# visinf/da-sac

Measured on AMD Instinct MI355X. Metric: train images/sec (769x769, 19-cls, RN101 DeepLabv2, K=3), higher is better.
Workload: dtype f32

## Files before the change

da-sac_amd/csrc/winograd.hip:

```cpp
#include "conv_common.hpp"
#include "winograd_index.hpp"

namespace dasac {
namespace wino {

constexpr int kBlock = 256;

__device__ __forceinline__ float ld(__amdgpu_buffer_rsrc_t r, unsigned voff) {
  return __uint_as_float(__builtin_amdgcn_raw_buffer_load_b32(r, voff, 0, 0));
}
__device__ __forceinline__ void st(__amdgpu_buffer_rsrc_t r, unsigned voff, float v) {
  __builtin_amdgcn_raw_buffer_store_b32(__float_as_uint(v), r, voff, 0, 0);
}

__global__ __launch_bounds__(kBlock) void filter_transform(const float* __restrict__ Wt, const float* __restrict__ scale,
                                                            float* __restrict__ U, int Cout, int Cin, int Mpad, int Kpad, int mode,
                                                            unsigned w_bytes, unsigned u_bytes) {
  const int idx = blockIdx.x * kBlock + threadIdx.x;
  const int per_point = Kpad * Mpad;
  if (idx >= per_point) return;
  const __amdgpu_buffer_rsrc_t rw = make_rsrc(Wt, w_bytes), ru = make_rsrc(U, u_bytes);
  const int row4 = Mpad * 4;
  const int kq = idx / row4, rem = idx - kq * row4;
  const int m = rem >> 2, k = kq * 4 + (rem & 3);
// ... 303 lines not shown
    float r[3][6];
#pragma unroll
    for (int b = 0; b < 6; ++b) {
      float p[6], o[3];
#pragma unroll
      for (int a = 0; a < 6; ++a) p[a] = (red[0][a * 6 + b][c] + red[1][a * 6 + b][c]) + (red[2][a * 6 + b][c] + red[3][a * 6 + b][c]);
      gt3(p[0], p[1], p[2], p[3], p[4], p[5], o);
#pragma unroll
      for (int a = 0; a < 3; ++a) r[a][b] = o[a];
    }
#pragma unroll
    for (int a = 0; a < 3; ++a) {
      float o[3];
      gt3(r[a][0], r[a][1], r[a][2], r[a][3], r[a][4], r[a][5], o);
#pragma unroll
      for (int b = 0; b < 3; ++b) grad[c * 9 + a * 3 + b] = o[b];
    }
  }
  __syncthreads();
  const float sc = scale ? ld(make_rsrc(scale, (unsigned)M * 4u), (unsigned)co * 4u) : 1.f;
  float part = 0.f;
  for (int e = tx; e < 64 * 9; e += kBlock) {
    const unsigned off = ((unsigned)(co * C + ci0) * 9u + (unsigned)e) * 4u;
    if (dot) part += grad[e] * ld(rw, off);
    st(rd, off, grad[e] * sc);
  }
  if (dot) {
    __shared__ float redd[4];
    part = wave_sum(part);
    if (c == 0) redd[q] = part;
    __syncthreads();
    if (tx == 0) st(make_rsrc(dot, (unsigned)((C / 64) * M) * 4u), (unsigned)(blockIdx.x * M + co) * 4u, (redd[0] + redd[1]) + (redd[2] + redd[3]));
  }
}

}
}

using namespace dasac;
using dasac::wino::Geom;

static int wino_geom(Geom& g, const char* who, int Nb, int C, int M, int H, int W, int dilation) {
  DASAC_REQUIRE(Nb > 0 && C > 0 && M > 0 && H > 0 && W > 0 && dilation > 0, "%s: bad geometry", who);
  DASAC_REQUIRE((int64_t)Nb * H * W < (1ll << 30), "%s: more than 2^30 pixels", who);
  g = wino::make_geom(Nb, H, W, dilation);
  const int64_t cmax = C > M ? C : M;
  DASAC_REQUIRE(16 * cmax * (int64_t)g.T * 4 <= wino::kMaxBytes && cmax * (int64_t)Nb * H * W * 4 <= wino::kMaxBytes,
                "%s: a tensor exceeds the 4 GiB buffer-descriptor window", who);
  return DASAC_OK;
}

extern "C" int dasac_winograd_tiles(int Nb, int H, int W, int dilation) {
  if (Nb <= 0 || H <= 0 || W <= 0 || dilation <= 0) return 0;
  const int64_t t = (int64_t)Nb * wino::make_axis(H, dilation).tiles * wino::make_axis(W, dilation).tiles;
  return t < (1ll << 30) ? (int)t : 0;
}

extern "C" int dasac_winograd_filter(const float* w, const float* scale, int Cout, int Cin, int transposed, float* u,
                                     dasac_stream_t stream) {
  DASAC_REQUIRE(w && u, "winograd_filter: null pointer");
  DASAC_REQUIRE(Cout > 0 && Cin > 0, "winograd_filter: bad channel counts");
  const int M = transposed ? Cin : Cout, K = transposed ? Cout : Cin;
  const int Mpad = dasac_conv_mpad(M), Kpad = dasac_conv_kpad(K);
  const int64_t per_point = (int64_t)Kpad * Mpad;
  DASAC_REQUIRE(16 * per_point * 4 <= wino::kMaxBytes && (int64_t)Cout * Cin * 9 * 4 <= wino::kMaxBytes,
                "winograd_filter: operand exceeds the 4 GiB buffer-descriptor window");
// ... 112 lines not shown
}

extern "C" int dasac_winograd4_grad_input(const float* dz, int Nb, int M, int H, int W, int dilation, float* dm, size_t dm_bytes,
                                          dasac_stream_t stream) {
  DASAC_REQUIRE(dz && dm, "winograd4_grad_input: null pointer");
  Geom g;
  const int rc = wino_geom4(g, "winograd4_grad_input", Nb, M, H, W, dilation);
  if (rc) return rc;
  const size_t need = (size_t)36 * M * g.T * 4;
  if (dm_bytes < need) return fail(DASAC_EWORKSPACE, "winograd4_grad_input: workspace too small (%zu < %zu)", dm_bytes, need);
  hipLaunchKernelGGL(wino::grad_transform4, dim3((g.T + wino::kBlock - 1) / wino::kBlock, M), dim3(wino::kBlock), 0, as_stream(stream), dz,
                     dm, g, M, (unsigned)((int64_t)Nb * M * H * W * 4), (unsigned)need);
  DASAC_CHECK_LAUNCH("winograd grad_transform4");
  return DASAC_OK;
}

extern "C" int dasac_winograd4_wgrad_finish(const void* workspace, size_t ws_bytes, int M, int C, int T, const float* w,
                                            const float* scale, float* dw, float* dot, float* sum_dz, dasac_stream_t stream) {
  DASAC_REQUIRE(workspace && w && dw, "winograd4_wgrad_finish: null pointer");
  DASAC_REQUIRE(M > 0 && M <= 65535 && C > 0 && C % 64 == 0, "winograd4_wgrad_finish: needs 1..65535 output channels and a multiple of 64 input channels");
  const int splits = dasac_conv_wgrad_batched_splits(36, M, C, T);
  DASAC_REQUIRE(splits > 0, "winograd4_wgrad_finish: the batched weight-gradient launch does not take this shape");
  const size_t need = dasac_conv_wgrad_batched_workspace(36, M, C, T);
  if (ws_bytes < need) return fail(DASAC_EWORKSPACE, "winograd4_wgrad_finish: workspace too small (%zu < %zu)", ws_bytes, need);
  const int64_t p_elems = (int64_t)splits * 36 * M * C;
  DASAC_REQUIRE(p_elems * 4 <= wino::kMaxBytes && (int64_t)M * C * 9 * 4 <= wino::kMaxBytes,
                "winograd4_wgrad_finish: a tensor exceeds the 4 GiB buffer-descriptor window");
  const float* P = reinterpret_cast<const float*>(workspace);
  hipLaunchKernelGGL(wino::wgrad_finish4, dim3(C / 64, M), dim3(wino::kBlock), 0, as_stream(stream), P, P + p_elems, splits, M, C, w, scale,
                     dw, dot, sum_dz, (unsigned)(p_elems * 4), (unsigned)((int64_t)M * C * 9 * 4));
  DASAC_CHECK_LAUNCH("winograd wgrad_finish4");
  return DASAC_OK;
}
```

da-sac_amd/csrc/winograd_index.hpp:

```cpp
#pragma once
#include <stdint.h>

#if defined(__HIPCC__)
#define DASAC_HD __host__ __device__ __forceinline__
#else
#define DASAC_HD inline
#endif

namespace dasac {
namespace wino {

struct Div {
  unsigned mul, shift;
  int d;
};
DASAC_HD Div make_div(int d) {
  Div f{0u, 0u, d < 1 ? 1 : d};
  if (d <= 1) return f;
  int l = 1;
  while ((1ll << l) < d) ++l;
  const unsigned long long p = 1ull << (31 + l);
  f.mul = (unsigned)((p + (unsigned)d - 1) / (unsigned)d);
  f.shift = (unsigned)(l - 1);
  return f;
// ... 70 lines not shown
}
template <int TM = 2>
DASAC_HD void tile_origin(const Geom& g, int tile, int& n, int& y0, int& x0) {
  n = div(tile, g.by_tiles_img);
  const int rem = tile - n * g.tiles_img;
  const int gy = div(rem, g.by_tx), gx = rem - gy * g.ax.tiles;
  int p, t;
  tile_decode(g.ay, gy, p, t);
  y0 = first_out<TM>(g.ay, p, t);
  tile_decode(g.ax, gx, p, t);
  x0 = first_out<TM>(g.ax, p, t);
}
DASAC_HD bool real_tile(const Geom& g, int tile) { return tile < g.N * g.tiles_img; }
template <int TM = 2>
DASAC_HD void pixel_tile(const Geom& g, int pix, int& n, int& rem, int& tile, int& ey, int& ex) {
  n = div(pix, g.by_hw);
  rem = pix - n * g.HW;
  const int y = div(rem, g.by_w), x = rem - y * g.W;
  int gy, gx;
  coord_to_tile<TM>(g.ay, y, gy, ey);
  coord_to_tile<TM>(g.ax, x, gx, ex);
  tile = (n * g.ay.tiles + gy) * g.ax.tiles + gx;
}

constexpr unsigned kOutside = 0xFFFFFFFFu;

DASAC_HD unsigned patch_offset(const Geom& g, int C, int n, int c, int y0, int x0, int ky, int kx) {
  const int y = y0 + (ky - 1) * g.ay.d, x = x0 + (kx - 1) * g.ax.d;
  if ((unsigned)y >= (unsigned)g.H || (unsigned)x >= (unsigned)g.W) return kOutside;
  return (unsigned)((n * C + c) * g.HW + y * g.W + x) * 4u;
}
DASAC_HD unsigned point_offset(const Geom& g, int C, int pt, int c, int tile) { return (unsigned)((pt * C + c) * g.T + tile) * 4u; }
DASAC_HD unsigned out_offset(const Geom& g, int M, int n, int m, int rem) { return (unsigned)((n * M + m) * g.HW + rem) * 4u; }
constexpr int64_t kMaxBytes = (1ll << 32) - 4096;

}
}
```

da-sac_amd/dasac_hip/engine.py:

```python
import torch

from . import ops
from . import lib as L


class ConvOp:
    kind = "conv"

    def __init__(self, src, dst, convs, bn, relu, res):
        c0 = convs[0]
        self.src, self.dst, self.res, self.relu = src, dst, res, bool(relu)
        self.convs, self.bn = list(convs), bn
        assert all(c.stride == c0.stride and c.in_channels == c0.in_channels and c.out_channels == c0.out_channels
                   and c.groups == 1 for c in convs)
        assert c0.stride[0] == c0.stride[1]
        branches = []
        for c in convs:
            assert c.dilation[0] == c.dilation[1] and c.padding[0] == c.padding[1]
            branches.append((c.kernel_size[0], c.kernel_size[1], c.dilation[0], c.padding[0]))
        self.spec = ops.ConvSpec(c0.in_channels, c0.out_channels, branches, c0.stride[0])
        self.has_bias = c0.bias is not None
        assert bn is None or len(convs) == 1
        self.expanded = ops.ExpandedConv(self.spec) if (len(convs) > 1 and c0.out_channels <= 32 and c0.stride[0] == 1) else None

# ... 25 lines not shown
        return self.expanded is None and len(self.convs) == 1

    def inputs(self):
        return [self.src] + ([self.res] if self.res is not None else [])

    def tensors(self, c, h, w):
        oh, ow = self.spec.out_hw(h, w)
        return ([(self.expanded.E, oh, ow)] if self.expanded is not None else []) + [(self.spec.cout, oh, ow)]

    def forward(self, eng, i, saved, keep):
        acts, spec = saved["acts"], self.spec
        xin = acts[self.src]
        Nb, _, H, W = xin.shape
        if self.expanded is not None:
            _, bias_sum, _ = eng.fold(self)
            return self.expanded.forward(xin, eng.packed(self, False), eng.table(self, H, W, False, xin.device), bias_sum)
        OH, OW = spec.out_hw(H, W)
        out = torch.empty((Nb, spec.cout, OH, OW), dtype=torch.float32, device=xin.device)
        res = None if self.res is None else acts[self.res]
        if self.bn is not None and self.bn.training:
            cb = self.convs[0].bias.detach() if self.has_bias else None
            ts = ops.tile_stats_buffer(Nb, spec.cout, OH, OW, xin.device) if ops.stats_ok(spec.cout, spec.cin) else None
            z = ops.conv_gemm(xin, eng.packed(self, False, None), eng.table(self, H, W, False, xin.device), out, (OH, OW),
                              spec.stride, spec.cout, spec.K, 1, cb, None, None, False, stats=ts)
            out, stats = ops.bn_train_forward(z, self.bn, res, self.relu, tile_stats=ts)
            if keep:
                saved["aux"][i] = (z, stats)
            return out
        scale, shift, _ = eng.fold(self)
        bits = None
        if keep and self.relu and eng._bits_wanted[self.dst] and ops.bits_ok(spec.cout, spec.cin):
            bits = ops.ReluBits(Nb, spec.cout, OH, OW, xin.device)
            saved["bits"][self.dst] = bits
        if res is None and ops.winograd_routed(spec, False, Nb, H, W):
            return ops.winograd_conv(xin, eng.winograd_filter(self, False, scale), out, spec.branches[0][2], shift, self.relu,
                                     bits_out=bits)
        return ops.conv_gemm(xin, eng.packed(self, False, scale), eng.table(self, H, W, False, xin.device), out, (OH, OW),
                             spec.stride, spec.cout, spec.K, 1, shift, res, None, self.relu, bits_out=bits)

    def backward(self, eng, bp, i, dz):
        spec, ex = self.spec, self.expanded
        xin = bp.acts[self.src]
        H, W = xin.shape[2:]
        dy_out = dz
        if ex is not None:
            d = ex.scatter(dz)
            self._param_grads_expanded(eng, bp, d, dz, xin)
        else:
            dz, scale = self._param_grads(eng, bp, i, dz, xin)
        if self.src != 0:
            relu = bp.arrive(self.src)
            if ex is not None:
                mask = bp.relu_pattern(self.src, spec.cin, ex.E) if relu else None
                bp.g[self.src] = ex.dgrad(d, eng.packed(self, True), eng.table(self, H, W, True, dz.device), (H, W),
                                          res=bp.g.get(self.src), mask=mask)
            else:
                mask = (bp.relu_pattern(self.src, spec.cin, spec.cout) if spec.stride == 1 else bp.acts[self.src]) if relu else None
                OH, OW = dz.shape[2:]
                if bp.g.get(self.src) is None and (mask is None or isinstance(mask, ops.ReluBits)) \
                        and ops.winograd_routed(spec, True, dz.shape[0], OH, OW):
                    dx = torch.empty((dz.shape[0], spec.cin, H, W), dtype=torch.float32, device=dz.device)
                    bp.g[self.src] = ops.winograd_conv(dz, eng.winograd_filter(self, True, scale), dx, spec.branches[0][2],
                                                       mask_bits=mask)
                else:
                    bp.g[self.src] = ops.conv_dgrad(spec, dz, None, (H, W), scale=scale, res=bp.g.get(self.src), mask=mask,
                                                    table=eng.table(self, OH, OW, True, dz.device),
                                                    packed=eng.packed(self, True, scale))
        if self.res is not None:
            bp.join(self.res, dy_out)
        if bp.sink is not None:
            bp.sink.done([j for j in self.pidx if bp.need[j]])

    def _param_grads_expanded(self, eng, bp, d, dz, xin):
        need = bp.need
        if any(need[j] for j in self.w_idx):
            bp.store(self.w_idx, self.expanded.wgrad(d, xin, [c.weight.detach() for c in self.convs],
                                                     eng.table(self, xin.shape[2], xin.shape[3], False, xin.device),
                                                     outs=[bp.dest(j) for j in self.w_idx]))
        if any(need[j] for j in self.b_idx):
            bp.fan_out(self.b_idx, ops.channel_sums(dz, out=bp.sums_dest(self.b_idx, True, self.spec.cout, dz.device)))

    def _param_grads(self, eng, bp, i, dz, xin):
        spec, need, grads = self.spec, bp.need, bp.grads
        w_idx, b_idx, bn_idx = self.w_idx, self.b_idx, self.bn_idx
        train_bn = i in bp.aux
        want_bias = any(need[j] for j in b_idx)
        want_bn = any(need[j] for j in bn_idx)
        if train_bn:
            z, stats = bp.aux.pop(i)
            dz, dg, db = ops.bn_train_backward(dz, z, stats, self.bn.weight.detach(), want_params=want_bn,
                                               outs=(bp.dest(bn_idx[0]), bp.dest(bn_idx[1])) if want_bn else (None, None))
            del z
            if want_bn:
# ... 343 lines not shown
    @staticmethod
    def _cached(store, slot, key, build, *args):
        ent = store.get(slot)
        if ent is None or ent[0] != key:
            ent = store[slot] = (key, build(None if ent is None else ent[1], *args), args)
        return ent[1]

    def fold(self, op):
        if op.bn is None and (not op.has_bias or len(op.convs) == 1):
            return None, (op.convs[0].bias.detach() if op.has_bias else None), None
        return self._cached(self._folds, id(op), _fold_key(op), self._build_fold, op)

    @staticmethod
    def _build_fold(old, op):
        if op.bn is None:
            acc = op.convs[0].bias.detach()
            for c in op.convs[1:]:
                acc = ops.add(acc, c.bias.detach())
            return None, acc, None
        bn = op.bn
        return ops.bn_fold(bn.weight.detach(), bn.bias.detach(), bn.running_mean, bn.running_var, bn.eps,
                           op.convs[0].bias.detach() if op.has_bias else None)

    def packed(self, op, transposed, scale=None):
        return self._cached(self._packs, (id(op), transposed), _pack_key(op, scale), self._build_pack, op, transposed, scale)

    @staticmethod
    def _build_pack(old, op, transposed, scale):
        weights = [c.weight.detach() for c in op.convs]
        if op.expanded is not None:
            return op.expanded.pack(weights, transposed, out=old)
        return ops.conv_pack(op.spec, weights, transposed, scale, out=old, order=ops.gemm_order(op.spec, transposed))

    def winograd_filter(self, op, transposed, scale=None):
        return self._cached(self._packs, (id(op), transposed, "winograd"), _pack_key(op, scale), self._build_winograd_filter,
                            op, transposed, scale)

    @staticmethod
    def _build_winograd_filter(old, op, transposed, scale):
        return ops.winograd_filter(op.spec, op.convs[0].weight.detach(), transposed, scale, out=old)

    def largest_tensor_bytes(self, Nb, H, W):
        shapes = {0: (None, H, W)}
        biggest = 0
        for op in self.plan.ops:
            made = op.tensors(*shapes[op.src])
            shapes[op.dst] = made[-1]
            biggest = max([biggest] + [Nb * (c or 1) * h * w * 4 for c, h, w in made])
        return biggest

    def _refresh_plan(self, device, transposed):
        bn_mode = tuple(bool(op.bn is not None and op.bn.training) for op in self._convs)
        key = (device.index, bool(transposed), bn_mode)
        plan = self._refresh.get(key)
        if plan is not None and plan["ptrs"] == self._refresh_ptrs():
            return plan
        lib = L.load()
        fold_jobs, pack_jobs, fold_ops, pack_slots = [], [], [], []
        for op in self._convs:
            if not op.refreshable:
                continue
            scale = None
            if op.frozen_bn:
                ent = self._fold_bufs.get(id(op))
                if ent is None:
                    C = op.spec.cout
                    ent = tuple(torch.empty(C, dtype=torch.float32, device=device) for _ in range(3))
                    self._fold_bufs[id(op)] = ent
                scale = ent[0]
                cb = op.convs[0].bias if op.has_bias else None
                fold_jobs.append((op.bn.weight, op.bn.bias, op.bn.running_mean, op.bn.running_var, cb, ent, op.bn.eps, op.spec.cout))
                fold_ops.append(op)
            for tr in ((False, True) if transposed else (False,)):
# ... 257 lines not shown
```

da-sac_amd/dasac_hip/lib.py:

```python
import ctypes as C
import os

import torch

LIB_PATH = os.environ.get("DASAC_LIB") or os.path.join(os.path.dirname(os.path.abspath(__file__)), "libdasac_hip.so")

_p, _i, _l, _f, _sz = C.c_void_p, C.c_int, C.c_int64, C.c_float, C.c_size_t

PROTOTYPES = {
    "dasac_version": (_i, []),
    "dasac_last_error": (C.c_char_p, []),
    "dasac_device_info": (_i, [C.POINTER(_i), C.POINTER(_i), C.c_char_p, _sz]),
    "dasac_reserved_cus": (_i, []),
    "dasac_set_reserved_cus": (_i, [_i]),
    "dasac_pseudo_labels_workspace": (_sz, [_i, _i, _l]),
    "dasac_pseudo_labels": (_i, [_p, _p, _p, _f, _f, _i, _i, _l, _p, _p, _p, _p, _sz, _p]),
    "dasac_conv_mpad": (_i, [_i]),
    "dasac_conv_kpad": (_i, [_i]),
    "dasac_conv_table": (_i, [_p, _p, _p, _p, _i, _i, _i, _i, _i, _i, _p, _p]),
    "dasac_conv_pack": (_i, [_p, _p, _i, _i, _i, _i, _i, _i, _i, _p, _p]),
    "dasac_relu_bits_words": (_sz, [_i, _l]),
    "dasac_conv_gemm_bits_ok": (_i, [_i, _i]),
    "dasac_conv_gemm": (_i, [_p, _p, _p, _p] + [_i] * 12 + [_p, _p, _p, _p, _p, _i, _i, _i, _i, _p, _sz, _p]),
    "dasac_conv_gemm_batched": (_i, [_p, _p, _p, _p] + [_i] * 12 + [_i, _l, _l, _l, _p]),
# ... 40 lines not shown
    "dasac_activation_stats": (_i, [_p, _i, _i, _i, _p, _i, _p, _sz, _p, _p]),
    "dasac_label_nodes": (_i, [_p, _i, _i, _i, _i, _i, _i, _i, _i, _p, _p]),
    "dasac_class_feature_stats_workspace": (_sz, [_i, _i, _i]),
    "dasac_class_feature_stats": (_i, [_p, _p, _i, _i, _i, _i, _p, _p, _p, _sz, _p]),
    "dasac_scale_planes": (_i, [_p, _p, _l, _l, _p, _p]),
    "dasac_add": (_i, [_p, _p, _p, _l, _p]),
    "dasac_relu_mask": (_i, [_p, _p, _p, _l, _p]),
    "dasac_bn_stats_workspace": (_sz, [_i, _i, _l]),
    "dasac_bn_stats": (_i, [_p, _i, _i, _l, _p, _p, _sz, _p]),
    "dasac_bn_train_finalize": (_i, [_p, C.c_double, _p, _p, _p, _p, _p, _p, _f, _f, _i, _p, _p, _p, _p, _p]),
    "dasac_bn_apply": (_i, [_p, _p, _p, _p, _i, _i, _i, _l, _p, _p]),
    "dasac_bn_bwd_reduce": (_i, [_p, _p, _p, _p, _i, _i, _l, _p, _p, _p, _p, _sz, _p]),
    "dasac_bn_train_finalize_tiles": (_i, [_p, _i, _i, C.c_double, _p, _p, _p, _p, _p, _f, _f, _i, _p, _p, _p, _p, _p]),
    "dasac_bn_tile_stats_reduce": (_i, [_p, _i, _i, _i, _p, _p]),
    "dasac_bn_train_apply_tiles": (_i, [_p, _p, _i, _i, C.c_double, _p, _p, _p, _p, _p, _f, _f, _p, _i, _i, _i, _l, _p, _p, _p, _p]),
    "dasac_bn_bwd_fused": (_i, [_p, _p, _p, _p, _p, C.c_double, _i, _i, _l, _p, _p, _p, _p, _sz, _p]),
    "dasac_conv_gemm_stats_ok": (_i, [_i, _i]),
    "dasac_conv_gemm_stats_tiles": (_i, [_i, _i, _i]),
    "dasac_conv_gemm_stats": (_i, [_p, _p, _p, _p] + [_i] * 12 + [_p, _p, _i, _i, _i, _i, _p, _sz, _p, _p]),
    "dasac_bn_bwd_apply": (_i, [_p, _p, _p, _p, _p, _p, C.c_double, _p, _i, _i, _l, _p, _p, _p, _p]),
    "dasac_winograd_tiles": (_i, [_i, _i, _i, _i]),
    "dasac_winograd_filter": (_i, [_p, _p, _i, _i, _i, _p, _p]),
    "dasac_winograd_input": (_i, [_p, _i, _i, _i, _i, _i, _p, _sz, _p]),
    "dasac_winograd_output": (_i, [_p, _sz, _i, _i, _i, _i, _i, _p, _i, _p, _p, _p, _p]),
    "dasac_winograd_grad_input": (_i, [_p, _i, _i, _i, _i, _i, _p, _sz, _p]),
    "dasac_conv_wgrad_batched_splits": (_i, [_i, _i, _i, _i]),
    "dasac_conv_wgrad_batched_workspace": (_sz, [_i, _i, _i, _i]),
    "dasac_conv_wgrad_batched": (_i, [_p, _p, _i, _i, _i, _i, _l, _l, _i, _p, _sz, _p]),
    "dasac_winograd_wgrad_finish": (_i, [_p, _sz, _i, _i, _i, _p, _p, _p, _p, _p, _p]),
    "dasac_winograd4_tiles": (_i, [_i, _i, _i, _i]),
    "dasac_winograd4_input": (_i, [_p, _i, _i, _i, _i, _i, _p, _sz, _p]),
    "dasac_winograd4_grad_input": (_i, [_p, _i, _i, _i, _i, _i, _p, _sz, _p]),
    "dasac_winograd4_wgrad_finish": (_i, [_p, _sz, _i, _i, _i, _p, _p, _p, _p, _p, _p]),
    "dasac_conv_pack_expanded":(_i, [_p, _i, _i, _i, _i, _i, _i, _i, _p, _p]),
    "dasac_tap_gather": (_i, [_p, _p, _p, _p, _p, _i, _i, _i, _p, _i, _i, _i, _p, _p]),
    "dasac_tap_scatter": (_i, [_p, _p, _p, _p, _p, _i, _i, _i, _i, _i, _i, _p, _p]),
    "dasac_conv_wgrad_finish_expanded": (_i, [_p, _i, _i, _i, _i, _i, _p, _i, _i, _i, _i, _p]),
    "dasac_pack_chunk_elems": (_i, []),
    "dasac_bn_fold_multi": (_i, [_p, _p, _i, _p]),
    "dasac_conv_pack_multi": (_i, [_p, _p, _i, _p]),
    "dasac_label_pad_mask": (_i, [_p, _p, _l, _i, _i, _p]),
    "dasac_dropout_planes": (_i, [C.c_uint64, C.c_uint64, _f, _l, _p, _p]),
    "dasac_iou_counts": (_i, [_p, _p, _i, _i, _l, _i, _p, _p]),
    "dasac_mask_counts": (_i, [_p, _p, _p, _p, _p, _p, _p, _i, _i, _l, _i, _p, _p]),
    "dasac_confusion_counts": (_i, [_p, _p, _p, _p, _p, _p, _i, _p, _i, _i, _l, _i, _p, _p, _i, _i, _p]),
    "dasac_view_consistency": (_i, [_p, _i, _i, _i, _l, _f, _p, _p, _p, _p]),
    "dasac_boundary_counts_workspace": (_sz, [_i, _i, _i, _i]),
    "dasac_boundary_counts": (_i, [_p, _p, _p, _p, _p, _p, _i, _p, _i, _i, _i, _i, _i, _i, _p, _p, _sz, _p]),
    "dasac_crf_meanfield_workspace": (_sz, [_i, _i, _i, _i, _i]),
    "dasac_crf_meanfield": (_i, [_p, _p, _i, _i, _i, _i, _i, _i, _i, _f, _f, _f, _f, _f, _f, _i, _p, _p, _p, _p, _p, _sz, _p]),
    "dasac_label_hist": (_i, [_p, _i, _l, _p, _p]),
    "dasac_make_views_table_ints": (_i, [_i, _i]),
    "dasac_make_views": (_i, [_p, _p, _p, _i, _i, _i, _p, _p, _p, _i, _p, _p, _p, _p]),
    "dasac_view_photometric_workspace": (_sz, [_i, _i, _i]),
    "dasac_view_photometric": (_i, [_p, _p, _i, _i, _i, _p, _p, _p, _i, _p, _p, _p, _sz, _p]),
    "dasac_conv_wgrad_dot_rows": (_i, [_i, _i]),
    "dasac_conv_wgrad_finish": (_i, [_p, _i, _i, _i, _i, _i, _p, _p, _p, _p, _p, _i, _i, _i, _p]),
    "dasac_crop_table_ints": (_i, [_i, _i]),
    "dasac_resize_u8": (_i, [_p, _l, _p, _l, _i, _p, _p, _l, _i, _p, _l, _p, _l, _p]),
    "dasac_make_crops": (_i, [_p, _l, _p, _l, _i, _p, _p, _l, _i, _i, _p, _p, _i, _p, _p, _p, _p, _p, _p]),
    "dasac_vis_panels": (_i, [_p, _p, _i, _i, _i, _i, _i, _p, _p, _p, _p, _p, _p, _p]),
    "dasac_vis_grid": (_i, [_p, _i, _i, _i, _i, _f, _p, _p]),
}


class VisJob(C.Structure):
# ... 106 lines not shown
```

da-sac_amd/dasac_hip/ops.py:

```python
import os

import torch

from . import lib as L


def _c(t):
    return t if t.is_contiguous() else t.contiguous()


class _Profile:

    def __init__(self):
        self.on, self.records = False, []

    def start(self):
        self.on, self.records = True, []

    def stop(self, by_shape=False):
        self.on = False
        torch.cuda.synchronize()
        out = {}
        for name, flops, a, b, tag, nbytes in self.records:
            d = out.setdefault((name, tag) if by_shape else name, {"flops": 0.0, "bytes": 0.0, "seconds": 0.0, "launches": 0})
# ... 307 lines not shown
    with PROFILE.span("winograd_output", 0.0, None, 4.0 * (y.numel() + out.numel())):
        L.check(lib.dasac_winograd_output(y.data_ptr(), y.numel() * 4, Nb, M, H, W, int(dilation), L.ptr(shift), int(relu),
                                          0 if mask_bits is None else mask_bits.words.data_ptr(),
                                          0 if bits_out is None else bits_out.words.data_ptr(), out.data_ptr(), L.stream_ptr()),
                "dasac_winograd_output")
    return out


def winograd_conv(x, u, out, dilation, shift=None, relu=False, mask_bits=None, bits_out=None, gemm_schedule="auto"):
    lib = L.load()
    L.require_gpu(x, u, out)
    Nb, C, H, W = x.shape
    M = out.shape[1]
    assert x.is_contiguous() and out.is_contiguous() and tuple(out.shape) == (Nb, M, H, W)
    assert tuple(u.shape) == (16, lib.dasac_conv_kpad(C), lib.dasac_conv_mpad(M)) and u.is_contiguous()
    T = lib.dasac_winograd_tiles(Nb, H, W, int(dilation))
    if T <= 0 or 64 * max(C, M) * T > _MAX_TENSOR_BYTES:
        raise L.DasacError("winograd_conv: [16, {}, tiles] exceeds the 4 GiB buffer-descriptor window".format(max(C, M)))
    v_elems, y_elems = 16 * C * T, 16 * M * T
    ws = L.workspace(4 * (v_elems + y_elems), x.device)[:4 * (v_elems + y_elems)].view(torch.float32)
    v, y = ws[:v_elems].view(16, C, T), ws[v_elems:v_elems + y_elems].view(16, M, T)
    with PROFILE.span("winograd_input", 0.0, None, 4.0 * (x.numel() + v_elems)):
        L.check(lib.dasac_winograd_input(x.data_ptr(), Nb, C, H, W, int(dilation), v.data_ptr(), v_elems * 4, L.stream_ptr()),
                "dasac_winograd_input")
    table = _winograd_table(C, T, x.device)
    if gemm_schedule == "auto" and lib.dasac_conv_mpad(M) % 128 != 0:
        gemm_schedule = None
    if gemm_schedule == "auto":
        conv_gemm_batched(v.view(16, 1, C, 1, T), u, table, y.view(16, 1, M, 1, T), (1, T), 1, M, C)
    else:
        for pt in range(16):
            conv_gemm(v[pt].view(1, C, 1, T), u[pt], table, y[pt].view(1, M, 1, T), (1, T), 1, M, C, schedule=gemm_schedule)
    return winograd_output(y, out, dilation, shift, relu, mask_bits, bits_out)


WINOGRAD_WGRAD_MIN_CHANNEL_PRODUCT = 256 * 256


def winograd_wgrad_routed(spec, Nb, H, W):
    if ALGORITHM != "auto" or not winograd_ok(spec) or spec.cin * spec.cout < WINOGRAD_WGRAD_MIN_CHANNEL_PRODUCT:
        return False
    lib = L.load()
    T = lib.dasac_winograd_tiles(Nb, H, W, spec.branches[0][2])
    return T > 0 and 64 * max(spec.cin, spec.cout) * T <= _MAX_TENSOR_BYTES \
        and lib.dasac_conv_wgrad_batched_splits(16, spec.cout, spec.cin, T) > 0


def winograd_wgrad(spec, dz, x, weight, scale=None, dot=None, sum_dz=None, out=None):
    lib = L.load()
    L.require_gpu(dz, x, weight, scale, dot, sum_dz)
    Nb, C, H, W = x.shape
    M, d = dz.shape[1], int(spec.branches[0][2])
    assert winograd_ok(spec) and (C, M) == (spec.cin, spec.cout) and tuple(dz.shape) == (Nb, M, H, W) and x.is_contiguous()
    assert dot is None or (tuple(dot.shape) == (dot_rows(spec), M) and dot.is_contiguous())
    T = lib.dasac_winograd_tiles(Nb, H, W, d)
    slab_bytes = lib.dasac_conv_wgrad_batched_workspace(16, M, C, T) if T > 0 else 0
    if slab_bytes == 0 or 64 * max(C, M) * T > _MAX_TENSOR_BYTES:
        raise L.DasacError("winograd_wgrad: {} x {} channels over {} tiles has no batched point contraction".format(M, C, T))
    v_elems, m_elems = 16 * C * T, 16 * M * T
    ws = L.workspace(4 * (v_elems + m_elems) + slab_bytes, x.device)
    v, dm, slabs = ws[:4 * v_elems], ws[4 * v_elems:4 * (v_elems + m_elems)], ws[4 * (v_elems + m_elems):]
    dz = _c(dz)
    with PROFILE.span("winograd_wgrad_input", 0.0, None, 4.0 * (x.numel() + v_elems)):
        L.check(lib.dasac_winograd_input(x.data_ptr(), Nb, C, H, W, d, v.data_ptr(), v.numel(), L.stream_ptr()), "dasac_winograd_input")
    with PROFILE.span("winograd_wgrad_grad", 0.0, None, 4.0 * (dz.numel() + m_elems)):
        L.check(lib.dasac_winograd_grad_input(dz.data_ptr(), Nb, M, H, W, d, dm.data_ptr(), dm.numel(), L.stream_ptr()),
# ... 1126 lines not shown
```

include/dasac_hip.h:

```cpp
#ifndef DASAC_HIP_H
#define DASAC_HIP_H

#include <stddef.h>
#include <stdint.h>

#ifdef __cplusplus
extern "C" {
#endif

#define DASAC_OK 0
#define DASAC_EINVAL (-1)
#define DASAC_EWORKSPACE (-2)
#define DASAC_ELAUNCH (-3)

typedef void* dasac_stream_t;

int dasac_version(void);
const char* dasac_last_error(void);
int dasac_device_info(int* cu_count, int* wave_size, char* arch, size_t arch_len);
int dasac_reserved_cus(void);
int dasac_set_reserved_cus(int n);

size_t dasac_pseudo_labels_workspace(int B, int C, int64_t HW);
int dasac_pseudo_labels(const float* probs, const uint8_t* ignore, const float* disc,
// ... 44 lines not shown
int dasac_conv_wgrad(const float* dz, const float* x, const int32_t* table,
                     int Nb, int Cx, int H, int W, int OH, int OW, int stride, int M, int K,
                     void* workspace, size_t ws_bytes, dasac_stream_t stream);
int dasac_conv_wgrad_x3(const float* dz, const float* x, const int32_t* table,
                        int Nb, int Cx, int H, int W, int OH, int OW, int stride, int M, int K,
                        void* workspace, size_t ws_bytes, dasac_stream_t stream);
int dasac_conv_wgrad_dot_rows(int Cin, int taps);
int dasac_conv_wgrad_finish(const void* workspace, int Nb, int OH, int OW, int M, int K,
                            const float* w, const float* scale, float* dw, float* dot,
                            float* sum_dz, int Cin, int taps, int tap0, dasac_stream_t stream);

int dasac_winograd_tiles(int Nb, int H, int W, int dilation);
int dasac_winograd_filter(const float* w, const float* scale, int Cout, int Cin, int transposed, float* u,
                          dasac_stream_t stream);
int dasac_winograd_input(const float* x, int Nb, int C, int H, int W, int dilation, float* v, size_t v_bytes,
                         dasac_stream_t stream);
int dasac_winograd_output(const float* y, size_t y_bytes, int Nb, int M, int H, int W, int dilation, const float* shift,
                          int relu, const uint32_t* mask_bits, uint32_t* relu_bits_out, float* out, dasac_stream_t stream);
int dasac_winograd_grad_input(const float* dz, int Nb, int M, int H, int W, int dilation, float* dm, size_t dm_bytes,
                              dasac_stream_t stream);
int dasac_conv_wgrad_batched_splits(int batch, int M, int C, int T);
size_t dasac_conv_wgrad_batched_workspace(int batch, int M, int C, int T);
int dasac_conv_wgrad_batched(const float* a, const float* b, int batch, int M, int C, int T, int64_t a_stride, int64_t b_stride,
                             int sum_entry, void* workspace, size_t ws_bytes, dasac_stream_t stream);
int dasac_winograd_wgrad_finish(const void* workspace, size_t ws_bytes, int M, int C, int T, const float* w, const float* scale,
                                float* dw, float* dot, float* sum_dz, dasac_stream_t stream);
int dasac_winograd4_tiles(int Nb, int H, int W, int dilation);
int dasac_winograd4_input(const float* x, int Nb, int C, int H, int W, int dilation, float* v, size_t v_bytes,
                          dasac_stream_t stream);
int dasac_winograd4_grad_input(const float* dz, int Nb, int M, int H, int W, int dilation, float* dm, size_t dm_bytes,
                               dasac_stream_t stream);
int dasac_winograd4_wgrad_finish(const void* workspace, size_t ws_bytes, int M, int C, int T, const float* w, const float* scale,
                                 float* dw, float* dot, float* sum_dz, dasac_stream_t stream);

int dasac_conv_pack_expanded(const float* w, int Cout, int Cin, int taps, int tap0, int total_taps,
                             int Cp, int transposed, float* packed, dasac_stream_t stream);
int dasac_tap_gather(const float* y, const int32_t* kh, const int32_t* kw, const int32_t* dil,
                     const int32_t* pad, int n_branches, int Cp, int Cout, const float* bias, int B,
                     int H, int W, float* out, dasac_stream_t stream);
int dasac_tap_scatter(const float* dout, const int32_t* kh, const int32_t* kw, const int32_t* dil,
                      const int32_t* pad, int n_branches, int Cp, int Cout, int B, int H, int W,
                      float* d, dasac_stream_t stream);
int dasac_conv_wgrad_finish_expanded(const void* workspace, int Nb, int OH, int OW, int E, int Cin,
                                     float* dw, int Cout, int taps, int tap0, int Cp,
                                     dasac_stream_t stream);

int dasac_upsample_softmax(const float* logits, int B, int C, int h, int w, int H, int W,
                           const uint8_t* ignore, float* up, float* probs, double* class_sums,
                           dasac_stream_t stream);
size_t dasac_upsample_bwd_workspace(int planes, int H, int w);
int dasac_upsample_bwd(const float* grad_up, int planes, int h, int w, int H, int W,
                       const float* gscale, float* grad_low, void* workspace, size_t ws_bytes,
                       dasac_stream_t stream);
size_t dasac_ce_loss_workspace(int B, int C, int64_t HW);
int dasac_ce_loss(const float* logits, const int64_t* labels, const float* class_weight,
                  const float* conf, int B, int C, int64_t HW, int mode, const float* gscale,
                  float* loss, float* dlogits, float* per_class, void* workspace, size_t ws_bytes,
                  dasac_stream_t stream);
size_t dasac_ce_loss_bwd_low_workspace(int B, int C, int H, int w);
int dasac_ce_loss_bwd_low(const float* logits_up, const int64_t* labels, const float* class_weight, const float* conf,
                          int B, int C, int H, int W, int h, int w, int mode, const float* gscale, float* grad_low,
                          void* workspace, size_t ws_bytes, dasac_stream_t stream);
int dasac_infer_labels(const float* logits, int B, int C, int h, int w, int H, int W, const uint8_t* lut,
                       uint8_t* labels, float* conf, dasac_stream_t stream);
#define DASAC_INFER_MAX_SOURCES 8
#define DASAC_INFER_MEAN 0
// ... 198 lines not shown
```

Measured before the change: 22.59.

## Route dilated 3x3 convs through F(4x4,3x3) Winograd forward and data-grad

Adds an F(4,3) Winograd path with 36 transform points: a filter transform kernel, an output transform kernel with shift/ReLU/mask epilogue, and a separate ReLU-bit packing kernel. Selected 512- and 256-channel dilated 3x3 convolutions in the forward and input-gradient passes are sent through this path, which uses a batched GEMM over the 36 points. The aim is to cut the multiply count relative to the F(2,3) path (16 points) for the large dilated ResNet layers. The cost is a larger transform workspace, an extra kernel pass when ReLU bits are recorded, and somewhat lower fp32 accuracy from the bigger transform constants.

New measurement: 23.55, median of 6. 1.04x the previous value.

```diff
diff --git a/da-sac_amd/csrc/winograd.hip b/da-sac_amd/csrc/winograd.hip
--- a/da-sac_amd/csrc/winograd.hip
+++ b/da-sac_amd/csrc/winograd.hip
@@ -359,6 +359,116 @@
     __syncthreads();
     if (tx == 0) st(make_rsrc(dot, (unsigned)((C / 64) * M) * 4u), (unsigned)(blockIdx.x * M + co) * 4u, (redd[0] + redd[1]) + (redd[2] + redd[3]));
   }
+}
+
+__device__ __forceinline__ void g6(float g0, float g1, float g2, float (&o)[6]) {
+  constexpr float k6 = 1.f / 6.f, k15 = 1.f / 15.f, k30 = 1.f / 30.f;
+  o[0] = 0.5f * g0;
+  o[1] = k6 * ((g0 + g2) + g1);
+  o[2] = k6 * ((g0 + g2) - g1);
+  o[3] = (k30 * g0 + k15 * g1) + (2.f * k15) * g2;
+  o[4] = ((16.f * k15) * g0 - (8.f * k15) * g1) + (4.f * k15) * g2;
+  o[5] = 0.5f * g2;
+}
+__device__ __forceinline__ void at4(float y0, float y1, float y2, float y3, float y4, float y5, float (&o)[4]) {
+  o[0] = (y0 + (y1 + y2)) + (y3 + y4);
+  o[1] = (y1 - y2) + (2.f * y3 - 0.5f * y4);
+  o[2] = (y1 + y2) + (4.f * y3 + 0.25f * y4);
+  o[3] = ((y1 - y2) + y5) + (8.f * y3 - 0.125f * y4);
+}
+
+__global__ __launch_bounds__(kBlock) void filter_transform4(const float* __restrict__ Wt, const float* __restrict__ scale,
+                                                             float* __restrict__ U, int Cout, int Cin, int Mpad, int Kpad, int mode,
+                                                             unsigned w_bytes, unsigned u_bytes) {
+  const int idx = blockIdx.x * kBlock + threadIdx.x;
+  const int per_point = Kpad * Mpad;
+  if (idx >= per_point) return;
+  const __amdgpu_buffer_rsrc_t rw = make_rsrc(Wt, w_bytes), ru = make_rsrc(U, u_bytes);
+  const int row4 = Mpad * 4;
+  const int kq = idx / row4, rem = idx - kq * row4;
+  const int m = rem >> 2, k = kq * 4 + (rem & 3);
+  const int M = mode == 0 ? Cout : Cin, K = mode == 0 ? Cin : Cout;
+  const bool real = m < M && k < K;
+  const int co = mode == 0 ? m : k, ci = mode == 0 ? k : m;
+  const float s = (real && scale) ? ld(make_rsrc(scale, (unsigned)Cout * 4u), (unsigned)co * 4u) : 1.f;
+  float t[6][3];
+#pragma unroll
+  for (int b = 0; b < 3; ++b) {
+    float g[3], o[6];
+#pragma unroll
+    for (int a = 0; a < 3; ++a) {
+      const int tap = mode == 0 ? a * 3 + b : (2 - a) * 3 + (2 - b);
+      g[a] = ld(rw, real ? (unsigned)((co * Cin + ci) * 9 + tap) * 4u : kOutside) * s;
+    }
+    g6(g[0], g[1], g[2], o);
+#pragma unroll
+    for (int a = 0; a < 6; ++a) t[a][b] = o[a];
+  }
+#pragma unroll
+  for (int a = 0; a < 6; ++a) {
+    float u[6];
+    g6(t[a][0], t[a][1], t[a][2], u);
+#pragma unroll
+    for (int b = 0; b < 6; ++b) st(ru, (unsigned)((a * 6 + b) * per_point + idx) * 4u, u[b]);
+  }
+}
+
+template <bool MASK>
+__global__ __launch_bounds__(kBlock) void output_transform4(const float* __restrict__ Y, float* __restrict__ Out, Geom g, int M,
+                                                             const float* __restrict__ shift, int relu,
+                                                             const unsigned* __restrict__ mbits, int w32, unsigned y_bytes,
+                                                             unsigned out_bytes, unsigned bits_bytes) {
+  const int tile = blockIdx.x * kBlock + threadIdx.x;
+  if (!real_tile(g, tile)) return;
+  const int m = blockIdx.y;
+  const __amdgpu_buffer_rsrc_t ry = make_rsrc(Y, y_bytes), ro = make_rsrc(Out, out_bytes);
+  int n, y0, x0;
+  tile_origin<4>(g, tile, n, y0, x0);
+  float t[4][6];
+#pragma unroll
+  for (int b = 0; b < 6; ++b) {
+    float v[6], o[4];
+#pragma unroll
+    for (int a = 0; a < 6; ++a) v[a] = ld(ry, point_offset(g, M, a * 6 + b, m, tile));
+    at4(v[0], v[1], v[2], v[3], v[4], v[5], o);
+#pragma unroll
+    for (int e = 0; e < 4; ++e) t[e][b] = o[e];
+  }
+  const float sh = shift ? ld(make_rsrc(shift, (unsigned)M * 4u), (unsigned)m * 4u) : 0.f;
+  const __amdgpu_buffer_rsrc_t rb = make_rsrc(mbits, MASK ? bits_bytes : 0u);
+#pragma unroll
+  for (int ey = 0; ey < 4; ++ey) {
+    float o[4];
+    at4(t[ey][0], t[ey][1], t[ey][2], t[ey][3], t[ey][4], t[ey][5], o);
+    const int y = y0 + ey * g.ay.d;
+#pragma unroll
+    for (int ex = 0; ex < 4; ++ex) {
+      const int x = x0 + ex * g.ax.d;
+      const bool in = y < g.H && x < g.W;
+      const int rem = y * g.W + x, pix = n * g.HW + rem;
+      float v = o[ex];
+      if (shift) v = v + sh;
+      if (relu) v = fmaxf(v, 0.f);
+      if constexpr (MASK) {
+        const unsigned word = __builtin_amdgcn_raw_buffer_load_b32(rb, in ? out_bits_offset(m, w32, pix) : kOutside, 0, 0);
+        v = (word >> (pix & 31)) & 1u ? v : 0.f;
+      }
+      st(ro, in ? out_offset(g, M, n, m, rem) : kOutside, v);
+    }
+  }
+}
+
+__global__ __launch_bounds__(kBlock) void relu_bits_pack(const float* __restrict__ Out, unsigned* __restrict__ obits, Geom g, int M,
+                                                          int w32, unsigned out_bytes, unsigned bits_bytes) {
+  const int pix = blockIdx.x * kBlock + threadIdx.x;
+  const int m = blockIdx.y;
+  const bool live = pix < g.N * g.HW;
+  const int n = live ? div(pix, g.by_hw) : 0;
+  const float v = ld(make_rsrc(Out, out_bytes), live ? out_offset(g, M, n, m, pix - n * g.HW) : kOutside);
+  const unsigned long long ballot = __builtin_amdgcn_ballot_w64(live && v > 0.f);
+  const int lane = threadIdx.x & 63, wcol = pix >> 5;
+  if ((lane & 31) == 0 && wcol < w32)
+    __builtin_amdgcn_raw_buffer_store_b32((unsigned)(lane ? ballot >> 32 : ballot), make_rsrc(obits, bits_bytes), out_bits_offset(m, w32, pix), 0, 0);
 }
 
 }
@@ -537,3 +647,50 @@
   DASAC_CHECK_LAUNCH("winograd wgrad_finish4");
   return DASAC_OK;
 }
+
+extern "C" int dasac_winograd4_filter(const float* w, const float* scale, int Cout, int Cin, int transposed, float* u,
+                                      dasac_stream_t stream) {
+  DASAC_REQUIRE(w && u, "winograd4_filter: null pointer");
+  DASAC_REQUIRE(Cout > 0 && Cin > 0, "winograd4_filter: bad channel counts");
+  const int M = transposed ? Cin : Cout, K = transposed ? Cout : Cin;
+  const int Mpad = dasac_conv_mpad(M), Kpad = dasac_conv_kpad(K);
+  const int64_t per_point = (int64_t)Kpad * Mpad;
+  DASAC_REQUIRE(36 * per_point * 4 <= wino::kMaxBytes && (int64_t)Cout * Cin * 9 * 4 <= wino::kMaxBytes,
+                "winograd4_filter: operand exceeds the 4 GiB buffer-descriptor window");
+  hipLaunchKernelGGL(wino::filter_transform4, dim3((unsigned)((per_point + wino::kBlock - 1) / wino::kBlock)), dim3(wino::kBlock), 0,
+                     as_stream(stream), w, scale, u, Cout, Cin, Mpad, Kpad, transposed ? 1 : 0, (unsigned)((int64_t)Cout * Cin * 9 * 4),
+                     (unsigned)(36 * per_point * 4));
+  DASAC_CHECK_LAUNCH("winograd filter_transform4");
+  return DASAC_OK;
+}
+
+extern "C" int dasac_winograd4_output(const float* y, size_t y_bytes, int Nb, int M, int H, int W, int dilation, const float* shift,
+                                      int relu, const uint32_t* mask_bits, uint32_t* relu_bits_out, float* out,
+                                      dasac_stream_t stream) {
+  DASAC_REQUIRE(y && out, "winograd4_output: null pointer");
+  DASAC_REQUIRE(!(mask_bits && relu_bits_out), "winograd4_output: record the ReLU pattern OR mask with one");
+  DASAC_REQUIRE(!relu_bits_out || relu, "winograd4_output: relu_bits_out records the pattern of a ReLU epilogue");
+  Geom g;
+  const int rc = wino_geom4(g, "winograd4_output", Nb, M, H, W, dilation);
+  if (rc) return rc;
+  const size_t need = (size_t)36 * M * g.T * 4;
+  if (y_bytes < need) return fail(DASAC_EWORKSPACE, "winograd4_output: workspace too small (%zu < %zu)", y_bytes, need);
+  const int npix = Nb * H * W, w32 = (npix + 31) / 32;
+  DASAC_REQUIRE((int64_t)M * w32 * 4 < (1ll << 31), "winograd4_output: bit mask exceeds 2 GiB");
+  const unsigned bits_bytes = (unsigned)((int64_t)M * w32 * 4), out_bytes = (unsigned)((int64_t)Nb * M * H * W * 4);
+  const dim3 grid((g.T + wino::kBlock - 1) / wino::kBlock, M), block(wino::kBlock);
+  hipStream_t s = as_stream(stream);
+  if (mask_bits)
+    hipLaunchKernelGGL(wino::output_transform4<true>, grid, block, 0, s, y, out, g, M, shift, relu, mask_bits, w32, (unsigned)need, out_bytes,
+                       bits_bytes);
+  else
+    hipLaunchKernelGGL(wino::output_transform4<false>, grid, block, 0, s, y, out, g, M, shift, relu, mask_bits, w32, (unsigned)need, out_bytes,
+                       bits_bytes);
+  if (relu_bits_out) {
+    DASAC_CHECK_LAUNCH("winograd output_transform4");
+    hipLaunchKernelGGL(wino::relu_bits_pack, dim3((npix + wino::kBlock - 1) / wino::kBlock, M), block, 0, s, out, relu_bits_out, g, M, w32,
+                       out_bytes, bits_bytes);
+  }
+  DASAC_CHECK_LAUNCH("winograd output_transform4");
+  return DASAC_OK;
+}
diff --git a/da-sac_amd/csrc/winograd_index.hpp b/da-sac_amd/csrc/winograd_index.hpp
--- a/da-sac_amd/csrc/winograd_index.hpp
+++ b/da-sac_amd/csrc/winograd_index.hpp
@@ -126,6 +126,7 @@
 }
 DASAC_HD unsigned point_offset(const Geom& g, int C, int pt, int c, int tile) { return (unsigned)((pt * C + c) * g.T + tile) * 4u; }
 DASAC_HD unsigned out_offset(const Geom& g, int M, int n, int m, int rem) { return (unsigned)((n * M + m) * g.HW + rem) * 4u; }
+DASAC_HD unsigned out_bits_offset(int m, int w32, int pix) { return (unsigned)(m * w32 + (pix >> 5)) * 4u; }
 constexpr int64_t kMaxBytes = (1ll << 32) - 4096;
 
 }
diff --git a/da-sac_amd/dasac_hip/engine.py b/da-sac_amd/dasac_hip/engine.py
--- a/da-sac_amd/dasac_hip/engine.py
+++ b/da-sac_amd/dasac_hip/engine.py
@@ -81,6 +81,9 @@
         if keep and self.relu and eng._bits_wanted[self.dst] and ops.bits_ok(spec.cout, spec.cin):
             bits = ops.ReluBits(Nb, spec.cout, OH, OW, xin.device)
             saved["bits"][self.dst] = bits
+        if res is None and ops.winograd4_routed(spec, False, Nb, H, W, keep):
+            return ops.winograd4_conv(xin, eng.winograd_filter(self, False, scale, points=36), out, spec.branches[0][2], shift,
+                                      self.relu, bits_out=bits)
         if res is None and ops.winograd_routed(spec, False, Nb, H, W):
             return ops.winograd_conv(xin, eng.winograd_filter(self, False, scale), out, spec.branches[0][2], shift, self.relu,
                                      bits_out=bits)
@@ -106,8 +109,12 @@
             else:
                 mask = (bp.relu_pattern(self.src, spec.cin, spec.cout) if spec.stride == 1 else bp.acts[self.src]) if relu else None
                 OH, OW = dz.shape[2:]
-                if bp.g.get(self.src) is None and (mask is None or isinstance(mask, ops.ReluBits)) \
-                        and ops.winograd_routed(spec, True, dz.shape[0], OH, OW):
+                wino_ok = bp.g.get(self.src) is None and (mask is None or isinstance(mask, ops.ReluBits))
+                if wino_ok and ops.winograd4_routed(spec, True, dz.shape[0], OH, OW, True):
+                    dx = torch.empty((dz.shape[0], spec.cin, H, W), dtype=torch.float32, device=dz.device)
+                    bp.g[self.src] = ops.winograd4_conv(dz, eng.winograd_filter(self, True, scale, points=36), dx, spec.branches[0][2],
+                                                        mask_bits=mask)
+                elif wino_ok and ops.winograd_routed(spec, True, dz.shape[0], OH, OW):
                     dx = torch.empty((dz.shape[0], spec.cin, H, W), dtype=torch.float32, device=dz.device)
                     bp.g[self.src] = ops.winograd_conv(dz, eng.winograd_filter(self, True, scale), dx, spec.branches[0][2],
                                                        mask_bits=mask)
@@ -517,13 +524,14 @@
             return op.expanded.pack(weights, transposed, out=old)
         return ops.conv_pack(op.spec, weights, transposed, scale, out=old, order=ops.gemm_order(op.spec, transposed))
 
-    def winograd_filter(self, op, transposed, scale=None):
-        return self._cached(self._packs, (id(op), transposed, "winograd"), _pack_key(op, scale), self._build_winograd_filter,
-                            op, transposed, scale)
-
-    @staticmethod
-    def _build_winograd_filter(old, op, transposed, scale):
-        return ops.winograd_filter(op.spec, op.convs[0].weight.detach(), transposed, scale, out=old)
+    def winograd_filter(self, op, transposed, scale=None, points=16):
+        slot = (id(op), transposed, "winograd") if points == 16 else (id(op), transposed, "winograd", points)
+        return self._cached(self._packs, slot, _pack_key(op, scale), self._build_winograd_filter, op, transposed, scale, points)
+
+    @staticmethod
+    def _build_winograd_filter(old, op, transposed, scale, points):
+        build = ops.winograd_filter if points == 16 else ops.winograd4_filter
+        return build(op.spec, op.convs[0].weight.detach(), transposed, scale, out=old)
 
     def largest_tensor_bytes(self, Nb, H, W):
         shapes = {0: (None, H, W)}
diff --git a/da-sac_amd/dasac_hip/lib.py b/da-sac_amd/dasac_hip/lib.py
--- a/da-sac_amd/dasac_hip/lib.py
+++ b/da-sac_amd/dasac_hip/lib.py
@@ -96,6 +96,8 @@
     "dasac_winograd4_input": (_i, [_p, _i, _i, _i, _i, _i, _p, _sz, _p]),
     "dasac_winograd4_grad_input": (_i, [_p, _i, _i, _i, _i, _i, _p, _sz, _p]),
     "dasac_winograd4_wgrad_finish": (_i, [_p, _sz, _i, _i, _i, _p, _p, _p, _p, _p, _p]),
+    "dasac_winograd4_filter": (_i, [_p, _p, _i, _i, _i, _p, _p]),
+    "dasac_winograd4_output": (_i, [_p, _sz, _i, _i, _i, _i, _i, _p, _i, _p, _p, _p, _p]),
     "dasac_conv_pack_expanded":(_i, [_p, _i, _i, _i, _i, _i, _i, _i, _p, _p]),
     "dasac_tap_gather": (_i, [_p, _p, _p, _p, _p, _i, _i, _i, _p, _i, _i, _i, _p, _p]),
     "dasac_tap_scatter": (_i, [_p, _p, _p, _p, _p, _i, _i, _i, _i, _i, _i, _p, _p]),
diff --git a/da-sac_amd/dasac_hip/ops.py b/da-sac_amd/dasac_hip/ops.py
--- a/da-sac_amd/dasac_hip/ops.py
+++ b/da-sac_amd/dasac_hip/ops.py
@@ -363,6 +363,77 @@
         for pt in range(16):
             conv_gemm(v[pt].view(1, C, 1, T), u[pt], table, y[pt].view(1, M, 1, T), (1, T), 1, M, C, schedule=gemm_schedule)
     return winograd_output(y, out, dilation, shift, relu, mask_bits, bits_out)
+
+
+WINOGRAD4_ROUTES = {
+    (512, 512, 4, True, True),
+    (512, 512, 4, False, False),
+    (256, 256, 2, False, False),
+}
+
+
+def winograd4_routed(spec, transposed, Nb, H, W, grad):
+    if ALGORITHM != "auto" or not winograd_ok(spec, transposed):
+        return False
+    d = spec.branches[0][2]
+    if (spec.cin, spec.cout, d, bool(transposed), bool(grad)) not in WINOGRAD4_ROUTES:
+        return False
+    lib = L.load()
+    if lib.dasac_conv_mpad(spec.cin if transposed else spec.cout) % 128:
+        return False
+    if H // d < WINOGRAD4_MIN_SAMPLES or W // d < WINOGRAD4_MIN_SAMPLES:
+        return False
+    T = lib.dasac_winograd4_tiles(Nb, H, W, d)
+    return T > 0 and 144 * max(spec.cin, spec.cout) * T <= _MAX_TENSOR_BYTES
+
+
+def winograd4_filter(spec, weight, transposed, scale=None, out=None):
+    lib = L.load()
+    L.require_gpu(weight, scale)
+    M, K = (spec.cin, spec.cout) if transposed else (spec.cout, spec.cin)
+    shape = (36, lib.dasac_conv_kpad(K), lib.dasac_conv_mpad(M))
+    if out is None or tuple(out.shape) != shape:
+        out = torch.empty(shape, dtype=torch.float32, device=weight.device)
+    L.check(lib.dasac_winograd4_filter(_c(weight).data_ptr(), L.ptr(scale), spec.cout, spec.cin, int(transposed), out.data_ptr(),
+                                       L.stream_ptr()), "dasac_winograd4_filter")
+    return out
+
+
+def winograd4_output(y, out, dilation, shift=None, relu=False, mask_bits=None, bits_out=None):
+    lib = L.load()
+    L.require_gpu(y, out, shift)
+    Nb, M, H, W = out.shape
+    assert y.is_contiguous() and out.is_contiguous() and y.dtype == torch.float32
+    for b in (mask_bits, bits_out):
+        assert b is None or b.shape == tuple(out.shape)
+    with PROFILE.span("winograd4_output", 0.0, None, 4.0 * (y.numel() + out.numel())):
+        L.check(lib.dasac_winograd4_output(y.data_ptr(), y.numel() * 4, Nb, M, H, W, int(dilation), L.ptr(shift), int(relu),
+                                           0 if mask_bits is None else mask_bits.words.data_ptr(),
+                                           0 if bits_out is None else bits_out.words.data_ptr(), out.data_ptr(), L.stream_ptr()),
+                "dasac_winograd4_output")
+    return out
+
+
+def winograd4_conv(x, u, out, dilation, shift=None, relu=False, mask_bits=None, bits_out=None):
+    lib = L.load()
+    L.require_gpu(x, u, out)
+    Nb, C, H, W = x.shape
+    M = out.shape[1]
+    assert x.is_contiguous() and out.is_contiguous() and tuple(out.shape) == (Nb, M, H, W)
+    assert tuple(u.shape) == (36, lib.dasac_conv_kpad(C), lib.dasac_conv_mpad(M)) and u.is_contiguous()
+    if lib.dasac_conv_mpad(M) % 128 != 0:
+        raise L.DasacError("winograd4_conv: {} output channels have no batched point GEMM".format(M))
+    T = lib.dasac_winograd4_tiles(Nb, H, W, int(dilation))
+    if T <= 0 or 144 * max(C, M) * T > _MAX_TENSOR_BYTES:
+        raise L.DasacError("winograd4_conv: [36, {}, tiles] exceeds the 4 GiB buffer-descriptor window".format(max(C, M)))
+    v_elems, y_elems = 36 * C * T, 36 * M * T
+    ws = L.workspace(4 * (v_elems + y_elems), x.device)[:4 * (v_elems + y_elems)].view(torch.float32)
+    v, y = ws[:v_elems].view(36, C, T), ws[v_elems:v_elems + y_elems].view(36, M, T)
+    with PROFILE.span("winograd4_input", 0.0, None, 4.0 * (x.numel() + v_elems)):
+        L.check(lib.dasac_winograd4_input(x.data_ptr(), Nb, C, H, W, int(dilation), v.data_ptr(), v_elems * 4, L.stream_ptr()),
+                "dasac_winograd4_input")
+    conv_gemm_batched(v.view(36, 1, C, 1, T), u, _winograd_table(C, T, x.device), y.view(36, 1, M, 1, T), (1, T), 1, M, C)
+    return winograd4_output(y, out, dilation, shift, relu, mask_bits, bits_out)
 
 
 WINOGRAD_WGRAD_MIN_CHANNEL_PRODUCT = 256 * 256
diff --git a/include/dasac_hip.h b/include/dasac_hip.h
--- a/include/dasac_hip.h
+++ b/include/dasac_hip.h
@@ -100,6 +100,10 @@
                                dasac_stream_t stream);
 int dasac_winograd4_wgrad_finish(const void* workspace, size_t ws_bytes, int M, int C, int T, const float* w, const float* scale,
                                  float* dw, float* dot, float* sum_dz, dasac_stream_t stream);
+int dasac_winograd4_filter(const float* w, const float* scale, int Cout, int Cin, int transposed, float* u,
+                           dasac_stream_t stream);
+int dasac_winograd4_output(const float* y, size_t y_bytes, int Nb, int M, int H, int W, int dilation, const float* shift,
+                           int relu, const uint32_t* mask_bits, uint32_t* relu_bits_out, float* out, dasac_stream_t stream);
 
 int dasac_conv_pack_expanded(const float* w, int Cout, int Cin, int taps, int tap0, int total_taps,
                              int Cp, int transposed, float* packed, dasac_stream_t stream);
```
